# CPJKU/beat_this

Hardware: AMD Instinct MI355X
Metric: audio-seconds processed/sec (higher is better)
Workload: dtype f32 activations, f16x3 products (3 x f16 MFMA on hi+lo operand halves, f32 accumulate); main-layer attention P.V: 2 x, probabilities as fp16 hi parts

## Files before the change

### beat_this_amd/csrc/gemm3.hip

```cpp

#include "common.h"
#include "kernels.h"

struct G3CfgS { static constexpr int BM = 128, BN = 128, BK = 32, WGM = 2, WGN = 2, NST = 3, OCC = 3; };
struct G3CfgB { static constexpr int BM = 256, BN = 256, BK = 64, WGM = 2, WGN = 4, NST = 2, OCC = 1; };
struct G3CfgT { static constexpr int BM = 192, BN = 256, BK = 64, WGM = 2, WGN = 4, NST = 2, OCC = 1; };
struct G3CfgSX { static constexpr int BM = 128, BN = 128, BK = 64, WGM = 2, WGN = 2, NST = 2, OCC = 2; };
struct G3CfgBX { static constexpr int BM = 256, BN = 256, BK = 64, WGM = 2, WGN = 4, NST = 2, OCC = 1; };
struct G3CfgTX { static constexpr int BM = 192, BN = 256, BK = 64, WGM = 2, WGN = 4, NST = 2, OCC = 1; };
struct G3CfgMX { static constexpr int BM = 256, BN = 128, BK = 32, WGM = 2, WGN = 2, NST = 3, OCC = 2; };
struct G3CfgHX { static constexpr int BM = 64, BN = 128, BK = 64, WGM = 2, WGN = 2, NST = 3, OCC = 2; };

#ifndef X3_NSPLIT
#define X3_NSPLIT 2
#endif

namespace {

typedef G3CfgS CfgS;
typedef G3CfgB CfgB;

constexpr unsigned OOB = 0x80000000u;

#ifndef BT_NT_STORE
#define BT_NT_STORE 1
#endif
#if BT_NT_STORE
#define ST_STREAM(ptr, val) __builtin_nontemporal_store((val), (ptr))
#else
#define ST_STREAM(ptr, val) (*(ptr) = (val))
#endif

typedef __amdgpu_buffer_rsrc_t rsrc_t;
typedef __attribute__((address_space(3))) void* lptr_t;
typedef __attribute__((ext_vector_type(4))) unsigned int u32x4;
typedef __attribute__((ext_vector_type(2))) unsigned int u32x2;

DEVI unsigned pk2(float a, float b) {
  const hfx2 t = {(hf)a, (hf)b};
  return __builtin_bit_cast(unsigned, t);
}

DEVI void pack_row_hf(const float (&v)[16], u32x4 (&piece)[2]) {
#pragma unroll
  for (int k = 0; k < 2; ++k) {
    unsigned x0 = pk2(v[8 * k], v[8 * k + 1]), x1 = pk2(v[8 * k + 2], v[8 * k + 3]);
    unsigned y0 = pk2(v[8 * k + 4], v[8 * k + 5]), y1 = pk2(v[8 * k + 6], v[8 * k + 7]);
    auto r0 = __builtin_amdgcn_permlane32_swap(x0, y0, false, false);
    auto r1 = __builtin_amdgcn_permlane32_swap(x1, y1, false, false);
    piece[k] = u32x4{r0[0], r1[0], r0[1], r1[1]};
  }
}

DEVI void split2(float a, float b, unsigned& whi, unsigned& wlo, float& amax) {
  split_hl(a, b, whi, wlo);
  amax = fmaxf(amax, fmaxf(fabsf(a), fabsf(b)));
}
DEVI void pack_row_hl(const float (&v)[16], u32x4 (&hi)[2], u32x4 (&lo)[2], float& amax) {
#pragma unroll
  for (int k = 0; k < 2; ++k) {
    unsigned xh[2], xl[2], yh[2], yl[2];
    split2(v[8 * k], v[8 * k + 1], xh[0], xl[0], amax);
    split2(v[8 * k + 2], v[8 * k + 3], xh[1], xl[1], amax);
    split2(v[8 * k + 4], v[8 * k + 5], yh[0], yl[0], amax);
    split2(v[8 * k + 6], v[8 * k + 7], yh[1], yl[1], amax);
    auto h0 = __builtin_amdgcn_permlane32_swap(xh[0], yh[0], false, false);
    auto h1 = __builtin_amdgcn_permlane32_swap(xh[1], yh[1], false, false);
    auto l0 = __builtin_amdgcn_permlane32_swap(xl[0], yl[0], false, false);
    auto l1 = __builtin_amdgcn_permlane32_swap(xl[1], yl[1], false, false);
    hi[k] = u32x4{h0[0], h1[0], h0[1], h1[1]};
    lo[k] = u32x4{l0[0], l1[0], l0[1], l1[1]};
  }
}
DEVI void pack_row_f8(const float (&v)[16], u32x4 (&hi)[2], u32x2 (&h8)[2], u32x2 (&l8)[2], float& amax) {
#pragma unroll
  for (int k = 0; k < 2; ++k) {
    unsigned xh[2], xl[2], yh[2], yl[2];
    split2(v[8 * k], v[8 * k + 1], xh[0], xl[0], amax);
    split2(v[8 * k + 2], v[8 * k + 3], xh[1], xl[1], amax);
    split2(v[8 * k + 4], v[8 * k + 5], yh[0], yl[0], amax);
    split2(v[8 * k + 6], v[8 * k + 7], yh[1], yl[1], amax);
    const unsigned x8 = pk4_f8(v[8 * k], v[8 * k + 1], v[8 * k + 2], v[8 * k + 3]);
    const unsigned y8 = pk4_f8(v[8 * k + 4], v[8 * k + 5], v[8 * k + 6], v[8 * k + 7]);
    const unsigned xl8 = lo4_f8(v[8 * k], v[8 * k + 1], v[8 * k + 2], v[8 * k + 3], xh[0], xh[1]);
    const unsigned yl8 = lo4_f8(v[8 * k + 4], v[8 * k + 5], v[8 * k + 6], v[8 * k + 7], yh[0], yh[1]);
    auto h0 = __builtin_amdgcn_permlane32_swap(xh[0], yh[0], false, false);
    auto h1 = __builtin_amdgcn_permlane32_swap(xh[1], yh[1], false, false);
    auto b8 = __builtin_amdgcn_permlane32_swap(x8, y8, false, false);
    auto c8 = __builtin_amdgcn_permlane32_swap(xl8, yl8, false, false);
    hi[k] = u32x4{h0[0], h1[0], h0[1], h1[1]};
    h8[k] = u32x2{b8[0], b8[1]};
    l8[k] = u32x2{c8[0], c8[1]};
  }
}
DEVI void flag_range(int* status, float amax, float limit = 65504.f) {
  if (status && __any(!(amax <= limit)) && (threadIdx.x & 63) == 0) atomicOr(status, 1);
}

#ifndef BT_QKV_GATE_TILE
#define BT_QKV_GATE_TILE 1
#endif
template <typename CFG>
DEVI void qkv_gate_tile_x3(const Gemm3P& p, char* smem, int m0, int n0, int n_tiles, int lane, int wave) {
  constexpr int BM = CFG::BM, BN = CFG::BN, ROWB = CFG::BK * 2, NST = CFG::NST, KR = CFG::BK / 2, EB = 4;
  constexpr int NW = CFG::WGM * CFG::WGN, NT = 64 * NW;
  constexpr int CPR = ROWB / 16, RPI = 64 / CPR;
  constexpr int A_BYTES = BM * ROWB, ST_BYTES = A_BYTES + BN * ROWB;
  constexpr int APC = A_BYTES / (NT * 16), LPS = APC + 1;
  static_assert(ROWB == 128 && NW * 32 == BM && 32 * ROWB == NT * 16 && APC <= 4, "one 32-token block per wave, one W piece per thread");
  const int g = lane >> 5, lr = lane & 31;
  const int nk = p.K / KR;
  const int Lv = p.nblk * 32;
  auto swz = [](int r) { return (r >> 1) & 7; };
  const unsigned a_bytes = (unsigned)((long)p.M * p.lda * EB), w_bytes = (unsigned)((long)n_tiles * BN * p.K * EB);
  unsigned voffA[4];
#pragma unroll
  for (int i = 0; i < APC; ++i) {
    const int r = (i * NW + wave) * RPI + lane / CPR;
    const int c = (lane % CPR) ^ swz(r);
    const long row = (long)m0 + r;
    const int seq = (int)(row / Lv), t = (int)(row - (long)seq * Lv);
    voffA[i] = (seq < p.n_seq && t < p.L) ? (unsigned)(((long)seq * p.L + t) * p.lda * EB + c * 16) : OOB;
  }
  unsigned voffW;
  {
    const int r = wave * RPI + lane / CPR;
    voffW = (unsigned)((long)(n0 + r) * p.K * EB + ((lane % CPR) ^ swz(r)) * 16);
  }
  const rsrc_t rA = __builtin_amdgcn_make_buffer_rsrc(const_cast<char*>(reinterpret_cast<const char*>(p.A)), 0, a_bytes, 0x00020000);
  const rsrc_t rW = __builtin_amdgcn_make_buffer_rsrc(const_cast<void*>(p.W), 0, w_bytes, 0x00020000);
  auto issue = [&](int kt, int stage) {
    char* st_ = smem + stage * ST_BYTES + wave * 1024;
    const int so_ = kt * ROWB;
#pragma unroll
    for (int i_ = 0; i_ < APC; ++i_)
      __builtin_amdgcn_raw_ptr_buffer_load_lds(rA, (lptr_t)(st_ + i_ * NW * 1024), 16, voffA[i_], so_, 0, 0);
    __builtin_amdgcn_raw_ptr_buffer_load_lds(rW, (lptr_t)(st_ + A_BYTES), 16, voffW, so_, 0, 0);
  };
  const int pofs = A_BYTES + lr * ROWB;
  const int qofs = (wave * 32 + lr) * ROWB;
  const int sw = swz(lr);
  int kc[4];
#pragma unroll
  for (int m = 0; m < 4; ++m) kc[m] = ((2 * m + g) ^ sw) * 16;
  f32x16 acc;
#pragma unroll
  for (int r = 0; r < 16; ++r) acc[r] = 0.f;
  const int vb = m0 + wave * 32;
  const int tseq = vb / Lv, tblk = (vb - tseq * Lv) >> 5;
  const int t = tblk * 32 + lr;
  const long trow = (tseq < p.n_seq && t < p.L) ? (long)tseq * p.L + t : -1;
  float part[8];
#pragma unroll
  for (int q = 0; q < 8; ++q) part[q] = (p.ssq_in && trow >= 0 && q < p.ssq_parts) ? p.ssq_in[(long)q * p.M + trow] : 0.f;
#pragma unroll
  for (int s0 = 0; s0 < NST - 1; ++s0)
    if (s0 < nk) issue(s0, s0);
  asm volatile("s_waitcnt vmcnt(0)" ::: "memory");
  __builtin_amdgcn_sched_barrier(0);
  float rs = 1.f;
  if (p.ssq_in) {
    float sum = 0.f;
#pragma unroll
    for (int q = 0; q < 8; ++q) sum += part[q];
    for (int q = 8; q < p.ssq_parts; ++q) sum += trow >= 0 ? p.ssq_in[(long)q * p.M + trow] : 0.f;
    rs = trow >= 0 ? sqrtf((float)p.K) / fmaxf(sqrtf(sum), 1e-12f) : 0.f;
  }
  int stage = 0, stage2 = NST - 1;
  for (int kt = 0; kt < nk; ++kt) {
    if (NST > 2 && kt + 1 < nk) asm volatile("s_waitcnt vmcnt(%0) lgkmcnt(0)" ::"n"((NST - 2) * LPS) : "memory");
    else asm volatile("s_waitcnt vmcnt(0) lgkmcnt(0)" ::: "memory");
    __builtin_amdgcn_s_barrier();
    if (kt + NST - 1 < nk) issue(kt + NST - 1, stage2);
    const char* st = smem + stage * ST_BYTES;
#pragma unroll
    for (int m = 0; m < 2; ++m) {
      const hfx8 ph = *reinterpret_cast<const hfx8*>(st + pofs + kc[m]);
      const hfx8 pl = *reinterpret_cast<const hfx8*>(st + pofs + kc[m + 2]);
      const hfx8 qh = *reinterpret_cast<const hfx8*>(st + qofs + kc[m]);
      const hfx8 ql = *reinterpret_cast<const hfx8*>(st + qofs + kc[m + 2]);
      acc = MFMA32_H(pl, qh, acc);
      acc = MFMA32_H(ph, ql, acc);
      acc = MFMA32_H(ph, qh, acc);
    }
    stage = stage == NST - 1 ? 0 : stage + 1;
    stage2 = stage2 == NST - 1 ? 0 : stage2 + 1;
  }
  if (tseq >= p.n_seq) return;
#pragma unroll
  for (int r = 0; r < 16; ++r) {
    const int h = n0 - 3 * p.inner + crow(r, g);
    if (h < p.heads) p.gates[((long)tseq * p.heads + h) * p.nbp * 32 + t] = sigmoidf(fmaf(acc[r], rs, p.b_gates[h]));
  }
}

template <int EPI, typename CFG, int X3 = 0>
__global__ __launch_bounds__(64 * CFG::WGM * CFG::WGN, (CFG::OCC * CFG::WGM * CFG::WGN + 3) / 4)
void gemm3_kernel(const Gemm3P p, int n_tiles, int total_tiles, int per_xcd, int nsplit) {
  constexpr int BM = CFG::BM, BN = CFG::BN, BK = CFG::BK, NST = CFG::NST;
  constexpr int NW = CFG::WGM * CFG::WGN, NT = 64 * NW;
  constexpr int TB = BM / CFG::WGM / 32;
  constexpr int FB = BN / CFG::WGN / 32;
  constexpr int ROWB = BK * 2;
  constexpr int KR = X3 ? BK / 2 : BK;
  constexpr bool HL16 = X3 && BK == 32;
  constexpr int EB = X3 ? 4 : 2;
  constexpr int CPR = ROWB / 16;
  constexpr int RPI = 64 / CPR;
  constexpr int A_BYTES = BM * ROWB, W_BYTES = BN * ROWB, ST_BYTES = A_BYTES + W_BYTES;
  constexpr int APC = A_BYTES / (NT * 16), WPC = W_BYTES / (NT * 16);
  static_assert(EPI != G3_QKV || TB == FB, "the V columns swap the operand roles: square wave tile needed");
  static_assert(BN / CFG::WGN == 64, "ssq partials are per 64 columns = one wave");
  static_assert(!X3 || ROWB == 128 || ROWB == 64, "hl32: a k-step is a whole group (128 B per row) or half of one (64 B)");
  static_assert(X3 != 2 || ROWB == 128, "hl8: a k-step is a whole 32-column group");
  static_assert(NST * ST_BYTES >= NW * 8192, "the epilogues stage 8 KB per wave in the ring's LDS");
  __shared__ __attribute__((aligned(16))) char smem[NST * ST_BYTES];
  const int bid = blockIdx.x;
  int m_tile, n_tile;
  if (nsplit <= 1) {
    const int tile = (bid & 7) * per_xcd + (bid >> 3);
    if (tile >= total_tiles) return;
    m_tile = tile / n_tiles;
    n_tile = tile - m_tile * n_tiles;
  } else {
    const int xcd = bid & 7, slot = bid >> 3;
    const int g = xcd % nsplit, j = xcd / nsplit, per_m = 8 / nsplit, nt = n_tiles / nsplit;
    const int m_local = slot / nt;
    m_tile = m_local * per_m + j;
    n_tile = g * nt + (slot - m_local * nt);
    if ((long)m_tile * n_tiles >= total_tiles) return;
  }
  const int m0 = m_tile * BM, n0 = n_tile * BN;
  const int tid = threadIdx.x, lane = tid & 63, wave = __builtin_amdgcn_readfirstlane(tid >> 6);
  const int g = lane >> 5, lr = lane & 31;
  const int wm = wave / CFG::WGN, wn = wave % CFG::WGN;
  const int nk = p.K / KR;
  auto swz = [](int r) { return ROWB == 64 ? (r >> 2) & 3 : (r >> 1) & 7; };
  const int Lv = p.nblk * 32;

  int kind = 0;
  if constexpr (EPI == G3_QKV) kind = n0 < 3 * p.inner ? n0 / p.inner : 3;
  const bool normal = EPI == G3_QKV && kind == 2;
  if constexpr (BT_QKV_GATE_TILE && EPI == G3_QKV && X3 == 1 && BM == 128 && BN == 128 && ROWB == 128 && NW == 4) {
    if (kind == 3 && p.heads <= 32 && (p.x3 & 15) != 3) {
      qkv_gate_tile_x3<CFG>(p, smem, m0, n0, n_tiles, lane, wave);
      return;
    }
  }

  const unsigned a_bytes = (unsigned)((long)p.M * p.lda * EB), w_bytes = (unsigned)((long)n_tiles * BN * p.K * EB);
  static_assert(APC >= 1 && WPC >= 1, "tile too small for the workgroup");
  static_assert(APC <= 4 && WPC <= 4, "voffA / voffW hold at most 4 pieces");
  unsigned voffA[4], voffW[4];
  int tapmask[4] = {0, 0, 0, 0};
#pragma unroll
  for (int i = 0; i < APC; ++i) {
    const int r = (i * NW + wave) * RPI + lane / CPR;
    const int c = (lane % CPR) ^ swz(r);
    long row = (long)m0 + r;
    bool ok = row < p.M;
    if constexpr (EPI == G3_QKV) {
      const int seq = (int)(row / Lv), t = (int)(row - (long)seq * Lv);
      ok = seq < p.n_seq && t < p.L;
      row = (long)seq * p.L + t;
    }
    voffA[i] = ok ? (unsigned)(row * p.lda * EB + (HL16 ? (c >> 1) * 64 + (c & 1) * 16 : c * 16)) : OOB;
    if constexpr (EPI == G3_RESID) {
      const int t = p.conv_C2 > 0 ? (int)((row / p.conv_F) % p.conv_T) : 1;
      tapmask[i] = ok ? ((t >= 1 ? 1 : 0) | 2 | (t + 1 < p.conv_T ? 4 : 0)) : 0;
    }
  }
#pragma unroll
  for (int i = 0; i < WPC; ++i) {
    const int r = (i * NW + wave) * RPI + lane / CPR;
    const int c = (lane % CPR) ^ swz(r);
    voffW[i] = (unsigned)((long)(n0 + r) * p.K * EB + (HL16 ? (c >> 1) * 64 + (c & 1) * 16 : c * 16));
  }
  const bool conv = EPI == G3_RESID && p.conv_C2 > 0;
  const unsigned tap_bytes = conv ? (unsigned)(p.conv_F * p.conv_C2 * EB) : 0u;
  const int c2_shift = conv ? __builtin_ctz((unsigned)p.conv_C2) : 0;
  const rsrc_t rA = __builtin_amdgcn_make_buffer_rsrc(const_cast<char*>(reinterpret_cast<const char*>(p.A)) - tap_bytes, 0,
                                                      a_bytes + 2 * tap_bytes, 0x00020000);
  const rsrc_t rW = __builtin_amdgcn_make_buffer_rsrc(const_cast<void*>(p.W), 0, w_bytes, 0x00020000);
#define G3_ISSUE(kt, stage)                                                                                          \
  do {                                                                                                                \
    char* st_ = smem + (stage) * ST_BYTES + wave * 1024;                                                              \
    const int so_ = HL16 ? ((kt) >> 1) * 128 + ((kt) & 1) * 32 : (kt) * ROWB;                                         \
    if (conv) {                                                                                                       \
      const int tap_ = ((kt) * KR) >> c2_shift;                                                                       \
      const int kin_ = ((kt) * KR) & (p.conv_C2 - 1);                                                                 \
      const int soa_ = tap_ * (int)tap_bytes + (HL16 ? (kin_ >> 5) * 128 + ((kin_ >> 4) & 1) * 32 : kin_ * EB);      \
      _Pragma("unroll") for (int i_ = 0; i_ < APC; ++i_)                                                              \
          __builtin_amdgcn_raw_ptr_buffer_load_lds(rA, (lptr_t)(st_ + i_ * NW * 1024), 16,                            \
                                                   ((tapmask[i_] >> tap_) & 1) ? voffA[i_] : OOB, soa_, 0, 0);        \
    } else {                                                                                                          \
      _Pragma("unroll") for (int i_ = 0; i_ < APC; ++i_)                                                              \
          __builtin_amdgcn_raw_ptr_buffer_load_lds(rA, (lptr_t)(st_ + i_ * NW * 1024), 16, voffA[i_], so_, 0, 0);     \
    }                                                                                                                 \
    _Pragma("unroll") for (int i_ = 0; i_ < WPC; ++i_)                                                                \
        __builtin_amdgcn_raw_ptr_buffer_load_lds(rW, (lptr_t)(st_ + A_BYTES + i_ * NW * 1024), 16, voffW[i_], so_, 0, 0); \
  } while (0)

  constexpr int NP = FB, NQ = TB;
  const int pofs = (normal ? wm * (TB * 32) * ROWB : A_BYTES + wn * (FB * 32) * ROWB) + lr * ROWB;
  const int qofs = (normal ? A_BYTES + wn * (FB * 32) * ROWB : wm * (TB * 32) * ROWB) + lr * ROWB;
  const int sw = swz(lr);
  constexpr int MS = ROWB / 32;
  int kc[MS];
#pragma unroll
  for (int m = 0; m < MS; ++m) kc[m] = ((2 * m + g) ^ sw) * 16;

  f32x16 acc[NP][NQ];
#pragma unroll
  for (int a = 0; a < NP; ++a)
#pragma unroll
    for (int b = 0; b < NQ; ++b)
#pragma unroll
      for (int r = 0; r < 16; ++r) acc[a][b][r] = 0.f;

  const int row0 = m0 + wm * (TB * 32);
  long trow[TB];
  int tseq[TB], tblk[TB];
#pragma unroll
  for (int j = 0; j < TB; ++j) {
    const long v = (long)row0 + 32 * j + lr;
    if constexpr (EPI == G3_QKV) {
      const int vb = row0 + 32 * j;
      tseq[j] = vb / Lv;
      tblk[j] = (vb - tseq[j] * Lv) >> 5;
      const int t = tblk[j] * 32 + lr;
      trow[j] = (tseq[j] < p.n_seq && t < p.L) ? (long)tseq[j] * p.L + t : -1;
    } else {
      tseq[j] = tblk[j] = 0;
      trow[j] = v < p.M ? v : -1;
    }
  }
  float rs[TB], part[TB][8];
#pragma unroll
  for (int j = 0; j < TB; ++j) {
    rs[j] = 1.f;
#pragma unroll
    for (int q = 0; q < 8; ++q)
      part[j][q] = (EPI != G3_RESID && p.ssq_in && trow[j] >= 0 && q < p.ssq_parts) ? p.ssq_in[(long)q * p.M + trow[j]] : 0.f;
  }
  f32x4 bqv[EPI == G3_FF1 ? FB : 1][4];
  if constexpr (EPI == G3_FF1) {
#pragma unroll
    for (int a = 0; a < FB; ++a)
#pragma unroll
      for (int q = 0; q < 4; ++q) bqv[a][q] = *reinterpret_cast<const f32x4*>(p.bias + n0 + wn * 64 + a * 32 + 8 * q + 4 * g);
  }
  f32x4 csv[EPI == G3_QKV ? TB : 1][4];
  if constexpr (EPI == G3_QKV) {
    if (kind < 2) {
#pragma unroll
      for (int b = 0; b < TB; ++b)
#pragma unroll
        for (int q = 0; q < 4; ++q)
          csv[b][q] = tseq[b] < p.n_seq ? *reinterpret_cast<const f32x4*>(p.rope + ((long)(tblk[b] * 32 + lr) * 16 + 4 * q + 2 * g) * 2)
                                        : f32x4{0.f, 0.f, 0.f, 0.f};
    }
  }
  constexpr int LPS = APC + WPC;
#pragma unroll
  for (int s0 = 0; s0 < NST - 1; ++s0)
    if (s0 < nk) G3_ISSUE(s0, s0);
  if (EPI == G3_FF1 || EPI == G3_QKV || (EPI != G3_RESID && p.ssq_in)) {
    asm volatile("s_waitcnt vmcnt(0)" ::: "memory");
    __builtin_amdgcn_sched_barrier(0);
  }
  if (EPI != G3_RESID && p.ssq_in) {
#pragma unroll
    for (int j = 0; j < TB; ++j) {
      float sum = 0.f;
#pragma unroll
      for (int q = 0; q < 8; ++q) sum += part[j][q];
      for (int q = 8; q < p.ssq_parts; ++q) sum += trow[j] >= 0 ? p.ssq_in[(long)q * p.M + trow[j]] : 0.f;
      rs[j] = trow[j] >= 0 ? sqrtf((float)p.K) / fmaxf(sqrtf(sum), 1e-12f) : 0.f;
    }
  }
  int stage = 0, stage2 = NST - 1;
  for (int kt = 0; kt < nk; ++kt) {
    long long tq0 = 0, tq1 = 0;
    if (NST > 2 && kt + 1 < nk) asm volatile("s_waitcnt vmcnt(%0) lgkmcnt(0)" ::"n"((NST - 2) * LPS) : "memory");
    else asm volatile("s_waitcnt vmcnt(0) lgkmcnt(0)" ::: "memory");
    __builtin_amdgcn_s_barrier();
    if (kt + NST - 1 < nk) G3_ISSUE(kt + NST - 1, stage2);
    const char* st = smem + stage * ST_BYTES;
    if constexpr (X3 == 2) {
      typedef __attribute__((ext_vector_type(8))) int i32x8;
      const int cP = 4 + 2 * g, cQ = 6 - 2 * g;
      const int kP0 = (cP ^ sw) * 16, kP1 = ((cP + 1) ^ sw) * 16, kQ0 = (cQ ^ sw) * 16, kQ1 = ((cQ + 1) ^ sw) * 16;
      {
        i32x8 p8[NP], q8[NQ];
#pragma unroll
        for (int a = 0; a < NP; ++a) {
          const u32x4 lo = *reinterpret_cast<const u32x4*>(st + pofs + a * 32 * ROWB + kP0);
          const u32x4 hi = *reinterpret_cast<const u32x4*>(st + pofs + a * 32 * ROWB + kP1);
          p8[a] = i32x8{(int)lo[0], (int)lo[1], (int)lo[2], (int)lo[3], (int)hi[0], (int)hi[1], (int)hi[2], (int)hi[3]};
        }
#pragma unroll
        for (int b = 0; b < NQ; ++b) {
          const u32x4 lo = *reinterpret_cast<const u32x4*>(st + qofs + b * 32 * ROWB + kQ0);
          const u32x4 hi = *reinterpret_cast<const u32x4*>(st + qofs + b * 32 * ROWB + kQ1);
          q8[b] = i32x8{(int)lo[0], (int)lo[1], (int)lo[2], (int)lo[3], (int)hi[0], (int)hi[1], (int)hi[2], (int)hi[3]};
        }
#pragma unroll
        for (int a = 0; a < NP; ++a)
#pragma unroll
          for (int b = 0; b < NQ; ++b)
            acc[a][b] = __builtin_amdgcn_mfma_scale_f32_32x32x64_f8f6f4(p8[a], q8[b], acc[a][b], 0, 0, 0, HL8_SCALE_WORD, 0, 0x7f7f7f7f);
      }
#pragma unroll
      for (int m = 0; m < 2; ++m) {
        hfx8 ph[NP], qh[NQ];
#pragma unroll
        for (int a = 0; a < NP; ++a) ph[a] = *reinterpret_cast<const hfx8*>(st + pofs + a * 32 * ROWB + kc[m]);
#pragma unroll
        for (int b = 0; b < NQ; ++b) qh[b] = *reinterpret_cast<const hfx8*>(st + qofs + b * 32 * ROWB + kc[m]);
#pragma unroll
        for (int a = 0; a < NP; ++a)
#pragma unroll
          for (int b = 0; b < NQ; ++b) acc[a][b] = MFMA32_H(ph[a], qh[b], acc[a][b]);
      }
    } else if constexpr (!X3) {
#pragma unroll
      for (int m = 0; m < MS; ++m) {
        hfx8 fp[NP], fq[NQ];
#pragma unroll
        for (int a = 0; a < NP; ++a) fp[a] = *reinterpret_cast<const hfx8*>(st + pofs + a * 32 * ROWB + kc[m]);
#pragma unroll
        for (int b = 0; b < NQ; ++b) fq[b] = *reinterpret_cast<const hfx8*>(st + qofs + b * 32 * ROWB + kc[m]);
#pragma unroll
        for (int a = 0; a < NP; ++a)
#pragma unroll
          for (int b = 0; b < NQ; ++b) acc[a][b] = MFMA32_H(fp[a], fq[b], acc[a][b]);
      }
    } else {
#pragma unroll
      for (int m = 0; m < MS / 2; ++m) {
        hfx8 ph[NP], pl[NP], qh[NQ], ql[NQ];
#pragma unroll
        for (int a = 0; a < NP; ++a) {
          ph[a] = *reinterpret_cast<const hfx8*>(st + pofs + a * 32 * ROWB + kc[m]);
          pl[a] = *reinterpret_cast<const hfx8*>(st + pofs + a * 32 * ROWB + kc[m + MS / 2]);
        }
#pragma unroll
        for (int b = 0; b < NQ; ++b) {
          qh[b] = *reinterpret_cast<const hfx8*>(st + qofs + b * 32 * ROWB + kc[m]);
          ql[b] = *reinterpret_cast<const hfx8*>(st + qofs + b * 32 * ROWB + kc[m + MS / 2]);
        }
#pragma unroll
        for (int a = 0; a < NP; ++a)
#pragma unroll
          for (int b = 0; b < NQ; ++b) acc[a][b] = MFMA32_H(pl[a], qh[b], acc[a][b]);
#pragma unroll
        for (int a = 0; a < NP; ++a)
#pragma unroll
          for (int b = 0; b < NQ; ++b) acc[a][b] = MFMA32_H(ph[a], ql[b], acc[a][b]);
#pragma unroll
        for (int a = 0; a < NP; ++a)
#pragma unroll
          for (int b = 0; b < NQ; ++b) acc[a][b] = MFMA32_H(ph[a], qh[b], acc[a][b]);
      }
    }
    stage = stage == NST - 1 ? 0 : stage + 1;
    stage2 = stage2 == NST - 1 ? 0 : stage2 + 1;
  }

#undef G3_ISSUE
  __syncthreads();
  char* wst = smem + wave * 8192;
  float amax = 0.f;
  if constexpr (EPI == G3_FF1 && X3) {
    char* out8 = reinterpret_cast<char*>(p.out);
    const int nb0 = n0 + wn * 64;
    const int r4 = lane >> 4, cp = lane & 15;
#pragma unroll
    for (int b = 0; b < TB; ++b) {
#pragma unroll
      for (int a = 0; a < FB; ++a) {
        float v[16];
#pragma unroll
        for (int r = 0; r < 16; ++r) v[r] = gelu_erf(fmaf(acc[a][b][r], rs[b], bqv[a][r >> 2][r & 3]));
        if (p.x3 & G3_X3_OUT_F8) {
          u32x4 hi[2];
          u32x2 h8[2], l8[2];
          pack_row_f8(v, hi, h8, l8, amax);
#pragma unroll
          for (int k = 0; k < 2; ++k) {
            *reinterpret_cast<u32x4*>(wst + lr * 256 + (((8 * a + 2 * k + g) ^ (lr & 15)) << 4)) = hi[k];
            *reinterpret_cast<u32x2*>(wst + lr * 256 + (((8 * a + 4 + k) ^ (lr & 15)) << 4) + 8 * g) = h8[k];
            *reinterpret_cast<u32x2*>(wst + lr * 256 + (((8 * a + 6 + k) ^ (lr & 15)) << 4) + 8 * g) = l8[k];
          }
        } else {
        u32x4 hi[2], lo[2];
        pack_row_hl(v, hi, lo, amax);
#pragma unroll
        for (int k = 0; k < 2; ++k) {
          *reinterpret_cast<u32x4*>(wst + lr * 256 + (((8 * a + 2 * k + g) ^ (lr & 15)) << 4)) = hi[k];
          *reinterpret_cast<u32x4*>(wst + lr * 256 + (((8 * a + 4 + 2 * k + g) ^ (lr & 15)) << 4)) = lo[k];
        }
        }
      }
      static_assert(FB == 2, "row = 64 features = 256 B of hl32");
#pragma unroll
      for (int ps = 0; ps < 8; ++ps) {
        const int r = ps * 4 + r4;
        const u32x4 w = *reinterpret_cast<const u32x4*>(wst + r * 256 + (cp << 4));
        const long row = (long)row0 + 32 * b + r;
        if (row < p.M) ST_STREAM(reinterpret_cast<u32x4*>(out8 + (row * p.ldo + nb0) * 4 + ((cp ^ (r & 15)) << 4)), w);
      }
    }
  } else if constexpr (EPI == G3_FF1) {
    hf* out = reinterpret_cast<hf*>(p.out);
    const int nb0 = n0 + wn * 64;
#pragma unroll
    for (int b = 0; b < TB; ++b) {
#pragma unroll
      for (int a = 0; a < FB; ++a) {
        float v[16];
#pragma unroll
        for (int r = 0; r < 16; ++r) v[r] = gelu_tanh(fmaf(acc[a][b][r], rs[b], bqv[a][r >> 2][r & 3]));
        u32x4 piece[2];
        pack_row_hf(v, piece);
#pragma unroll
        for (int k = 0; k < 2; ++k)
          *reinterpret_cast<u32x4*>(wst + lr * 128 + (((4 * a + 2 * k + g) ^ (lr & 7)) << 4)) = piece[k];
      }
      static_assert(FB == 2, "row = 64 features = 128 B");
#pragma unroll
      for (int ps = 0; ps < 4; ++ps) {
        const int r = ps * 8 + (lane >> 3), cp = lane & 7;
        const u32x4 w = *reinterpret_cast<const u32x4*>(wst + r * 128 + (cp << 4));
        const long row = (long)row0 + 32 * b + r;
        if (row < p.M) *reinterpret_cast<u32x4*>(out + row * p.ldo + nb0 + ((cp ^ (r & 7)) << 3)) = w;
      }
    }
  } else if constexpr (EPI == G3_RESID) {
    hf* xb = reinterpret_cast<hf*>(p.xb);
    const int nb0 = n0 + wn * 64;
    if (nb0 < p.N) {
    if (p.bias) {
#pragma unroll
      for (int a = 0; a < FB; ++a)
#pragma unroll
        for (int q = 0; q < 4; ++q) {
          const f32x4 bb = *reinterpret_cast<const f32x4*>(p.bias + nb0 + a * 32 + 8 * q + 4 * g);
#pragma unroll
          for (int b = 0; b < TB; ++b)
#pragma unroll
            for (int i = 0; i < 4; ++i) acc[a][b][4 * q + i] += bb[i];
        }
    }
    const int r4 = lane >> 4, cp = lane & 15;
    const unsigned ldx = (unsigned)p.ldx;
    const unsigned off_lane = (unsigned)(row0 + r4) * ldx + (unsigned)nb0;
    unsigned colq[4];
#pragma unroll
    for (int q = 0; q < 4; ++q) colq[q] = (unsigned)((cp ^ (4 * q + r4)) << 2);
    const int rows_left = p.M - row0 - r4;
    if (p.gelu) {
#pragma unroll
      for (int a = 0; a < FB; ++a)
#pragma unroll
        for (int b = 0; b < TB; ++b)
#pragma unroll
          for (int r = 0; r < 16; ++r) acc[a][b][r] = X3 ? gelu_erf(acc[a][b][r]) : gelu_tanh(acc[a][b][r]);
    }
#pragma unroll
    for (int b = 0; b < TB; ++b) {
      f32x4 xv[8];
#pragma unroll
      for (int ps = 0; ps < 8; ++ps) {
        const unsigned off = off_lane + (unsigned)(32 * b + 4 * ps) * ldx + colq[ps & 3];
        xv[ps] = (32 * b + 4 * ps < rows_left && !p.no_resid && p.x) ? *reinterpret_cast<const f32x4*>(p.x + off)
                                                               : f32x4{0.f, 0.f, 0.f, 0.f};
      }
#pragma unroll
      for (int a = 0; a < FB; ++a)
#pragma unroll
        for (int q = 0; q < 4; ++q)
          *reinterpret_cast<f32x4*>(wst + lr * 256 + (((8 * a + 2 * q + g) ^ (lr & 15)) << 4)) =
              f32x4{acc[a][b][4 * q], acc[a][b][4 * q + 1], acc[a][b][4 * q + 2], acc[a][b][4 * q + 3]};
#pragma unroll
      for (int ps = 0; ps < 8; ++ps) {
        const int r = ps * 4 + r4;
        const unsigned off = off_lane + (unsigned)(32 * b + 4 * ps) * ldx + colq[ps & 3];
        const bool ok = 32 * b + 4 * ps < rows_left;
        f32x4 v = *reinterpret_cast<const f32x4*>(wst + r * 256 + (cp << 4));
#pragma unroll
        for (int i = 0; i < 4; ++i) v[i] += xv[ps][i];
        if (ok) {
          if (p.x) *reinterpret_cast<f32x4*>(p.x + off) = v;
          if constexpr (X3) {
            if (xb) {
              const unsigned f = (unsigned)nb0 + colq[ps & 3];
              unsigned wh[2], wl[2];
              split2(v[0], v[1], wh[0], wl[0], amax);
              split2(v[2], v[3], wh[1], wl[1], amax);
              hf* d = xb + (2u * off - (f & 31u));
              *reinterpret_cast<u32x2*>(d) = u32x2{wh[0], wh[1]};
              if (p.x3 & G3_X3_OUT_F8) {
                char* gb = reinterpret_cast<char*>(d) - (f & 31u);
                *reinterpret_cast<unsigned*>(gb + 64) = pk4_f8(v[0], v[1], v[2], v[3]);
                *reinterpret_cast<unsigned*>(gb + 96) = lo4_f8(v[0], v[1], v[2], v[3], wh[0], wh[1]);
              } else {
                *reinterpret_cast<u32x2*>(d + 32) = u32x2{wl[0], wl[1]};
              }
            }
          } else {
            if (xb) *reinterpret_cast<u32x2*>(xb + off) = u32x2{pk2(v[0], v[1]), pk2(v[2], v[3])};
          }
        }
        if (p.ssq_out) {
          float ssq = ok ? fmaf(v[0], v[0], fmaf(v[1], v[1], fmaf(v[2], v[2], v[3] * v[3]))) : 0.f;
#pragma unroll
          for (int o = 8; o > 0; o >>= 1) ssq += __shfl_xor(ssq, o);
          if (ok && cp == 0) p.ssq_out[(unsigned)(n0 / 64 + wn) * (unsigned)p.M + (unsigned)(row0 + 32 * b + r)] = ssq;
        }
      }
    }
    }
  } else {
    constexpr int BLK_E = X3 ? 2048 : 1024;
    if (kind < 2) {
      hf* dst = reinterpret_cast<hf*>(kind == 0 ? p.qf : p.kf);
#pragma unroll
      for (int b = 0; b < TB; ++b) {
        if (tseq[b] >= p.n_seq) continue;
        const f32x4 (&cs)[4] = csv[b];
#pragma unroll
        for (int a = 0; a < FB; ++a) {
          const int head = (n0 - kind * p.inner + wn * 64 + a * 32) >> 5;
          hf* blk = dst + (((long)tseq[b] * p.heads + head) * p.nbp + tblk[b]) * BLK_E;
#pragma unroll
          for (int q = 0; q < 4; ++q) {
            const float e0 = acc[a][b][4 * q] * rs[b], o0 = acc[a][b][4 * q + 1] * rs[b];
            const float e1 = acc[a][b][4 * q + 2] * rs[b], o1 = acc[a][b][4 * q + 3] * rs[b];
            const float r0 = e0 * cs[q][0] - o0 * cs[q][1], r1 = o0 * cs[q][0] + e0 * cs[q][1];
            const float r2 = e1 * cs[q][2] - o1 * cs[q][3], r3 = o1 * cs[q][2] + e1 * cs[q][3];
            if constexpr (X3) {
              unsigned wh[2], wl[2];
              split2(r0, r1, wh[0], wl[0], amax);
              split2(r2, r3, wh[1], wl[1], amax);
              ST_STREAM(reinterpret_cast<u32x2*>(blk + (q * 32 + lr) * 8 + 4 * g), (u32x2{wh[0], wh[1]}));
              ST_STREAM(reinterpret_cast<u32x2*>(blk + 1024 + (q * 32 + lr) * 8 + 4 * g), (u32x2{wl[0], wl[1]}));
            } else {
              *reinterpret_cast<u32x2*>(blk + (q * 32 + lr) * 8 + 4 * g) = u32x2{pk2(r0, r1), pk2(r2, r3)};
            }
          }
        }
      }
    } else if (kind == 2) {
      hf* dst = reinterpret_cast<hf*>(p.vf);
#pragma unroll
      for (int a = 0; a < TB; ++a) {
        if (tseq[a] >= p.n_seq) continue;
        float sk[16];
#pragma unroll
        for (int r = 0; r < 16; ++r) sk[r] = __shfl(rs[a], crow(r, g));
#pragma unroll
        for (int b = 0; b < FB; ++b) {
          const int head = (n0 - 2 * p.inner + wn * 64 + b * 32) >> 5;
          hf* blk = dst + (((long)tseq[a] * p.heads + head) * p.nbp + tblk[a]) * BLK_E;
#pragma unroll
          for (int s = 0; s < 2; ++s) {
            unsigned w[4], wl[4] = {0, 0, 0, 0};
#pragma unroll
            for (int i = 0; i < 4; ++i) {
              const float v0 = acc[a][b][8 * s + 2 * i] * sk[8 * s + 2 * i], v1 = acc[a][b][8 * s + 2 * i + 1] * sk[8 * s + 2 * i + 1];
              if constexpr (X3) split2(v0, v1, w[i], wl[i], amax);
              else w[i] = pk2(v0, v1);
            }
            ST_STREAM(reinterpret_cast<u32x4*>(blk + (s * 64 + lane) * 8), (u32x4{w[0], w[1], w[2], w[3]}));
            if constexpr (X3) ST_STREAM(reinterpret_cast<u32x4*>(blk + 1024 + (s * 64 + lane) * 8), (u32x4{wl[0], wl[1], wl[2], wl[3]}));
          }
        }
      }
    } else {
#pragma unroll
      for (int b = 0; b < TB; ++b) {
        if (tseq[b] >= p.n_seq) continue;
        const int t = tblk[b] * 32 + lr;
#pragma unroll
        for (int a = 0; a < FB; ++a)
#pragma unroll
          for (int r = 0; r < 16; ++r) {
            const int h = n0 - 3 * p.inner + wn * 64 + a * 32 + crow(r, g);
            if (h < p.heads)
              p.gates[((long)tseq[b] * p.heads + h) * p.nbp * 32 + t] = sigmoidf(fmaf(acc[a][b][r], rs[b], p.b_gates[h]));
          }
      }
    }
  }
  if constexpr (X3) flag_range(p.status, amax, (p.x3 & G3_X3_OUT_F8) ? HL8_ACT_MAX : 65504.f);
}

template <int EPI, typename CFG, int X3 = 0>
void launch_cfg(const Gemm3P& p, hipStream_t s) {
  const int n_tiles = (p.N + CFG::BN - 1) / CFG::BN;
  const long rows = p.epi == G3_QKV ? (long)p.n_seq * p.nblk * 32 : (long)p.M;
  const long m_tiles = (rows + CFG::BM - 1) / CFG::BM;
  const long total = m_tiles * n_tiles;
  int nsplit = (p.x3 >> 4) & 15;
  if (nsplit == 0) nsplit = (X3 && X3_NSPLIT > 1 && (long)n_tiles * CFG::BN * p.K * 4 > (5L << 19) && n_tiles % X3_NSPLIT == 0) ? X3_NSPLIT : 1;
  if (nsplit != 2 && nsplit != 4 && nsplit != 8) nsplit = 1;
  if (n_tiles % nsplit) nsplit = 1;
  long per;
  if (nsplit == 1) {
    per = (total + 7) / 8;
    per = (per + n_tiles - 1) / n_tiles * n_tiles;
  } else {
    const long per_m = 8 / nsplit;
    per = (m_tiles + per_m - 1) / per_m * (n_tiles / nsplit);
  }
  dim3 grid((unsigned)(per * 8)), block(64 * CFG::WGM * CFG::WGN);
  hipLaunchKernelGGL((gemm3_kernel<EPI, CFG, X3>), grid, block, 0, s, p, n_tiles, (int)total, (int)per, nsplit);
}

}

bool gemm3_supported(const Gemm3P& p) {
  const int eb = p.x3 ? 4 : 2;
  if (p.M <= 0 || p.K % 64 != 0 || p.K < 128 || p.lda % 8 != 0) return false;
  if ((long)p.M * p.lda * eb >= 0x7fffffffL || (long)(p.N + 255) / 256 * 256 * p.K * eb >= 0x7fffffffL) return false;
  if (p.x3 && BT_HALF_IS_BF16) return false;
  if (p.conv_C2 > 0 && (p.epi != G3_RESID || (p.conv_C2 & (p.conv_C2 - 1)) || p.conv_C2 % 32 != 0 || p.lda != p.conv_C2 ||
                        p.K != 3 * p.conv_C2 || p.conv_F <= 0 || p.conv_T <= 0 || p.M % (p.conv_T * p.conv_F) != 0 || !p.no_resid))
    return false;
  if (p.epi == G3_RESID && !p.x && !p.xb) return false;
  if (p.epi == G3_QKV) return p.inner % 128 == 0 && p.inner == p.heads * 32 && p.L > 0 && (long)p.n_seq * ((p.L + 31) / 32 * 32) < 0x7fffffffL;
  if (p.epi == G3_FF1) return p.N % 128 == 0 && p.ldo % 8 == 0;
  if (p.epi == G3_RESID) return p.N % 64 == 0 && p.ldx % 8 == 0 && (long)(p.M + 256) * p.ldx * (p.x3 ? 2 : 1) < 0x7fffffffL &&
                                (long)(p.N / 64) * p.M < 0x7fffffffL;
  return false;
}

#ifndef X3_BIG_FF1
#define X3_BIG_FF1 0
#endif
#ifndef X3_MX
#define X3_MX 1
#endif

int launch_gemm3(const Gemm3P& p, hipStream_t s) {
  if (!gemm3_supported(p)) return -2;
  const bool big_ok = p.epi != G3_QKV && p.N % 256 == 0;
  const int force = (p.x3 & 15) == 2 ? 1 : (p.x3 & 15) == 3 ? 0 : -1;
  const bool forced_small = (p.x3 & 15) == 4 || (p.x3 & 15) == 5;
  const long tiles192 = ((long)p.M + 191) / 192 * (p.N / 256);
  const bool fills = !p.x3 || tiles192 >= 160;
  const bool big = big_ok && !forced_small && (force == 1 || (force != 0 && p.epi == G3_RESID && p.K >= 1024 && p.M >= 4096 && fills) ||
                              (force != 0 && p.x3 && X3_BIG_FF1 && p.epi == G3_FF1 && p.M >= 4096));
  auto cost = [&](int bm) { const long t = ((long)p.M + bm - 1) / bm * (p.N / 256); return (t + 255) / 256 * bm; };
  const bool rows192 = big && p.epi == G3_RESID && force != 1 && cost(192) < cost(256);
  const long mx_tiles = ((long)p.M + 255) / 256 * ((p.N + 127) / 128);
  const bool f8 = (p.x3 & G3_X3_F8) != 0;
  const bool mx = p.x3 && !f8 && p.epi != G3_QKV && !big && !rows192 && force != 0 &&
                  ((p.x3 & 15) == 4 || (X3_MX && mx_tiles >= 512 && p.M >= 20000));
  const long sx_tiles = ((long)p.M + 127) / 128 * ((p.N + 127) / 128);
  const bool hx = p.x3 && p.epi == G3_RESID && !big && !rows192 && !mx &&
                  ((p.x3 & 15) == 5 || ((p.x3 & 15) <= 1 && (sx_tiles < 256 || (p.K < 1024 && p.M < 20000))));
  if (p.x3) {
    if (f8) {
      if (p.epi == G3_QKV) launch_cfg<G3_QKV, G3CfgSX, 2>(p, s);
      else if (p.epi == G3_FF1) { if (big) launch_cfg<G3_FF1, G3CfgBX, 2>(p, s); else launch_cfg<G3_FF1, G3CfgSX, 2>(p, s); }
      else if (hx) launch_cfg<G3_RESID, G3CfgHX, 2>(p, s);
      else if (rows192) launch_cfg<G3_RESID, G3CfgTX, 2>(p, s);
      else if (big) launch_cfg<G3_RESID, G3CfgBX, 2>(p, s);
      else launch_cfg<G3_RESID, G3CfgSX, 2>(p, s);
      return (int)hipGetLastError();
    }
    switch (p.epi) {
      case G3_FF1:
        if (mx) launch_cfg<G3_FF1, G3CfgMX, true>(p, s);
        else if (big) launch_cfg<G3_FF1, G3CfgBX, true>(p, s); else launch_cfg<G3_FF1, G3CfgSX, true>(p, s);
        break;
      case G3_RESID:
        if (mx) launch_cfg<G3_RESID, G3CfgMX, true>(p, s);
        else if (hx) launch_cfg<G3_RESID, G3CfgHX, true>(p, s);
        else if (rows192) launch_cfg<G3_RESID, G3CfgTX, true>(p, s);
        else if (big) launch_cfg<G3_RESID, G3CfgBX, true>(p, s);
        else launch_cfg<G3_RESID, G3CfgSX, true>(p, s);
        break;
      case G3_QKV: launch_cfg<G3_QKV, G3CfgSX, true>(p, s); break;
      default: return -1;
    }
    return (int)hipGetLastError();
  }
  switch (p.epi) {
    case G3_FF1:
      if (big) launch_cfg<G3_FF1, CfgB>(p, s);
      else launch_cfg<G3_FF1, CfgS>(p, s);
      break;
    case G3_RESID:
      if (rows192) launch_cfg<G3_RESID, G3CfgT>(p, s);
      else if (big) launch_cfg<G3_RESID, CfgB>(p, s);
      else launch_cfg<G3_RESID, CfgS>(p, s);
      break;
    case G3_QKV: launch_cfg<G3_QKV, CfgS>(p, s); break;
    default: return -1;
  }
  return (int)hipGetLastError();
}
```

Baseline: 63670.

## Add phased ping-pong main loop for big f16x3 GEMM tiles

Adds a phased main loop for the 256x256 and 192x256 hl32 GEMM configs. The two wave rows are offset by a barrier, and each k-step is split into four MFMA phases between barriers, with LDS reads and split global-to-LDS loads interleaved and MFMAs run at raised priority. Row blocks are interleaved across wave rows so each 64-row A piece is loaded per phase, and the epilogue row mapping changes to match. It also changes the dispatch heuristics: a new cost threshold for choosing 192-row tiles, FF1 can route to the phased configs, and the big-FF1 M threshold rises. This aims to overlap memory traffic and LDS reads with matrix math, at the cost of more barriers and tighter register and scheduling constraints.

Measured after the change: 64280 (median of 6 runs). About the same (+0.9%).

```diff
diff --git a/beat_this_amd/csrc/gemm3.hip b/beat_this_amd/csrc/gemm3.hip
--- a/beat_this_amd/csrc/gemm3.hip
+++ b/beat_this_amd/csrc/gemm3.hip
@@ -8,6 +8,11 @@
 struct G3CfgSX { static constexpr int BM = 128, BN = 128, BK = 64, WGM = 2, WGN = 2, NST = 2, OCC = 2; };
 struct G3CfgBX { static constexpr int BM = 256, BN = 256, BK = 64, WGM = 2, WGN = 4, NST = 2, OCC = 1; };
 struct G3CfgTX { static constexpr int BM = 192, BN = 256, BK = 64, WGM = 2, WGN = 4, NST = 2, OCC = 1; };
+struct G3CfgBP : G3CfgBX {};
+struct G3CfgTP : G3CfgTX {};
+template <typename CFG> struct G3Phased { static constexpr bool value = false; };
+template <> struct G3Phased<G3CfgBP> { static constexpr bool value = true; };
+template <> struct G3Phased<G3CfgTP> { static constexpr bool value = true; };
 struct G3CfgMX { static constexpr int BM = 256, BN = 128, BK = 32, WGM = 2, WGN = 2, NST = 3, OCC = 2; };
 struct G3CfgHX { static constexpr int BM = 64, BN = 128, BK = 64, WGM = 2, WGN = 2, NST = 3, OCC = 2; };
 
@@ -209,6 +214,10 @@
   constexpr int RPI = 64 / CPR;
   constexpr int A_BYTES = BM * ROWB, W_BYTES = BN * ROWB, ST_BYTES = A_BYTES + W_BYTES;
   constexpr int APC = A_BYTES / (NT * 16), WPC = W_BYTES / (NT * 16);
+  constexpr bool PH = G3Phased<CFG>::value;
+  static_assert(!PH || (X3 == 1 && ROWB == 128 && NST == 2 && CFG::WGM == 2 && CFG::WGN == 4 && FB == 2 && (TB == 3 || TB == 4) &&
+                        APC == TB && WPC == 4 && (EPI == G3_FF1 || EPI == G3_RESID)),
+                "phased loop: hl32 operands, 8 waves as 2 x 4, a 64-row A piece per token-block pair, FF1 / RESID");
   static_assert(EPI != G3_QKV || TB == FB, "the V columns swap the operand roles: square wave tile needed");
   static_assert(BN / CFG::WGN == 64, "ssq partials are per 64 columns = one wave");
   static_assert(!X3 || ROWB == 128 || ROWB == 64, "hl32: a k-step is a whole group (128 B per row) or half of one (64 B)");
@@ -318,12 +327,13 @@
 #pragma unroll
       for (int r = 0; r < 16; ++r) acc[a][b][r] = 0.f;
 
-  const int row0 = m0 + wm * (TB * 32);
+  const int row0 = PH ? m0 : m0 + wm * (TB * 32);
+  auto brow = [&](int b) { return PH ? 32 * (b < 2 ? 2 * wm + b : 4 + (TB - 2) * wm + (b - 2)) : 32 * b; };
   long trow[TB];
   int tseq[TB], tblk[TB];
 #pragma unroll
   for (int j = 0; j < TB; ++j) {
-    const long v = (long)row0 + 32 * j + lr;
+    const long v = (long)row0 + brow(j) + lr;
     if constexpr (EPI == G3_QKV) {
       const int vb = row0 + 32 * j;
       tseq[j] = vb / Lv;
@@ -362,10 +372,31 @@
     }
   }
   constexpr int LPS = APC + WPC;
+#define G3_ISSUE_A(kt, stage, i_)                                                                                     \
+  __builtin_amdgcn_raw_ptr_buffer_load_lds(rA, (lptr_t)(smem + (stage) * ST_BYTES + wave * 1024 + (i_) * NW * 1024), 16, voffA[i_], \
+                                           (kt) * ROWB, 0, 0)
+#define G3_ISSUE_W(kt, stage, i_)                                                                                     \
+  __builtin_amdgcn_raw_ptr_buffer_load_lds(rW, (lptr_t)(smem + (stage) * ST_BYTES + wave * 1024 + A_BYTES + (i_) * NW * 1024), 16, \
+                                           voffW[i_], (kt) * ROWB, 0, 0)
+  if constexpr (PH) {
+#pragma unroll
+    for (int i = 0; i < 2; ++i) G3_ISSUE_A(0, 0, i);
+#pragma unroll
+    for (int i = 0; i < 4; ++i) G3_ISSUE_W(0, 0, i);
+#pragma unroll
+    for (int i = 2; i < APC; ++i) G3_ISSUE_A(0, 0, i);
+    if (nk > 1) {
+#pragma unroll
+      for (int i = 0; i < 2; ++i) G3_ISSUE_A(1, 1, i);
+#pragma unroll
+      for (int i = 0; i < 4; ++i) G3_ISSUE_W(1, 1, i);
+    }
+  } else {
 #pragma unroll
   for (int s0 = 0; s0 < NST - 1; ++s0)
     if (s0 < nk) G3_ISSUE(s0, s0);
-  if (EPI == G3_FF1 || EPI == G3_QKV || (EPI != G3_RESID && p.ssq_in)) {
+  }
+  if (PH || EPI == G3_FF1 || EPI == G3_QKV || (EPI != G3_RESID && p.ssq_in)) {
     asm volatile("s_waitcnt vmcnt(0)" ::: "memory");
     __builtin_amdgcn_sched_barrier(0);
   }
@@ -379,6 +410,98 @@
       rs[j] = trow[j] >= 0 ? sqrtf((float)p.K) / fmaxf(sqrtf(sum), 1e-12f) : 0.f;
     }
   }
+  if constexpr (PH) {
+    constexpr int NL = APC - 2;
+    const int wofs = A_BYTES + (wn * 64 + lr) * ROWB;
+    int aofs[TB];
+#pragma unroll
+    for (int b = 0; b < TB; ++b) aofs[b] = (brow(b) + lr) * ROWB;
+    hfx8 wh[2][FB], wl[2][FB], qh[2][2], ql[2][2];
+    auto rd_w = [&](const char* st, int m) __attribute__((always_inline)) {
+#pragma unroll
+      for (int a = 0; a < FB; ++a) {
+        wh[m][a] = *reinterpret_cast<const hfx8*>(st + wofs + a * 32 * ROWB + kc[m]);
+        wl[m][a] = *reinterpret_cast<const hfx8*>(st + wofs + a * 32 * ROWB + kc[m + 2]);
+      }
+    };
+    auto rd_a = [&](const char* st, int h, int m) __attribute__((always_inline)) {
+#pragma unroll
+      for (int bb = 0; bb < 2; ++bb)
+        if (2 * h + bb < TB) {
+          qh[m][bb] = *reinterpret_cast<const hfx8*>(st + aofs[2 * h + bb] + kc[m]);
+          ql[m][bb] = *reinterpret_cast<const hfx8*>(st + aofs[2 * h + bb] + kc[m + 2]);
+        }
+    };
+    auto mm = [&](int h, int m) __attribute__((always_inline)) {
+      __builtin_amdgcn_sched_barrier(0);
+      asm volatile("s_waitcnt lgkmcnt(0)" ::: "memory");
+      __builtin_amdgcn_s_barrier();
+      __builtin_amdgcn_sched_barrier(0);
+      __builtin_amdgcn_s_setprio(1);
+#pragma unroll
+      for (int a = 0; a < FB; ++a)
+#pragma unroll
+        for (int bb = 0; bb < 2; ++bb)
+          if (2 * h + bb < TB) acc[a][2 * h + bb] = MFMA32_H(wl[m][a], qh[m][bb], acc[a][2 * h + bb]);
+#pragma unroll
+      for (int a = 0; a < FB; ++a)
+#pragma unroll
+        for (int bb = 0; bb < 2; ++bb)
+          if (2 * h + bb < TB) acc[a][2 * h + bb] = MFMA32_H(wh[m][a], ql[m][bb], acc[a][2 * h + bb]);
+#pragma unroll
+      for (int a = 0; a < FB; ++a)
+#pragma unroll
+        for (int bb = 0; bb < 2; ++bb)
+          if (2 * h + bb < TB) acc[a][2 * h + bb] = MFMA32_H(wh[m][a], qh[m][bb], acc[a][2 * h + bb]);
+      __builtin_amdgcn_s_setprio(0);
+      __builtin_amdgcn_sched_barrier(0);
+      __builtin_amdgcn_s_barrier();
+      __builtin_amdgcn_sched_barrier(0);
+    };
+    __builtin_amdgcn_s_barrier();
+    if (wm == 1) __builtin_amdgcn_s_barrier();
+    __builtin_amdgcn_sched_barrier(0);
+    rd_w(smem, 0);
+    rd_a(smem, 0, 0);
+    for (int kt = 0; kt < nk; ++kt) {
+      const int s = kt & 1;
+      const char* st = smem + s * ST_BYTES;
+      rd_w(st, 1);
+      rd_a(st, 0, 1);
+      if (kt + 1 < nk) {
+#pragma unroll
+        for (int i = 2; i < APC; ++i) G3_ISSUE_A(kt + 1, s ^ 1, i);
+        asm volatile("s_waitcnt vmcnt(%0)" ::"n"(APC + 4) : "memory");
+      } else {
+        asm volatile("s_waitcnt vmcnt(0)" ::: "memory");
+      }
+      mm(0, 0);
+      rd_a(st, 1, 0);
+      mm(0, 1);
+      rd_a(st, 1, 1);
+      if (kt + 2 < nk) {
+#pragma unroll
+        for (int i = 0; i < 2; ++i) G3_ISSUE_A(kt + 2, s, i);
+#pragma unroll
+        for (int i = 0; i < 2; ++i) G3_ISSUE_W(kt + 2, s, i);
+        asm volatile("s_waitcnt vmcnt(%0)" ::"n"(APC + 2) : "memory");
+      } else if (kt + 1 < nk) {
+        asm volatile("s_waitcnt vmcnt(%0)" ::"n"(NL) : "memory");
+      }
+      mm(1, 0);
+      if (kt + 1 < nk) {
+        rd_w(smem + (s ^ 1) * ST_BYTES, 0);
+        rd_a(smem + (s ^ 1) * ST_BYTES, 0, 0);
+      }
+      if (kt + 2 < nk) {
+#pragma unroll
+        for (int i = 2; i < 4; ++i) G3_ISSUE_W(kt + 2, s, i);
+      }
+      mm(1, 1);
+    }
+    asm volatile("s_waitcnt lgkmcnt(0)" ::: "memory");
+    if (wm == 0) __builtin_amdgcn_s_barrier();
+  } else {
   int stage = 0, stage2 = NST - 1;
   for (int kt = 0; kt < nk; ++kt) {
     long long tq0 = 0, tq1 = 0;
@@ -467,8 +590,11 @@
     stage = stage == NST - 1 ? 0 : stage + 1;
     stage2 = stage2 == NST - 1 ? 0 : stage2 + 1;
   }
+  }
 
 #undef G3_ISSUE
+#undef G3_ISSUE_A
+#undef G3_ISSUE_W
   __syncthreads();
   char* wst = smem + wave * 8192;
   float amax = 0.f;
@@ -508,7 +634,7 @@
       for (int ps = 0; ps < 8; ++ps) {
         const int r = ps * 4 + r4;
         const u32x4 w = *reinterpret_cast<const u32x4*>(wst + r * 256 + (cp << 4));
-        const long row = (long)row0 + 32 * b + r;
+        const long row = (long)row0 + brow(b) + r;
         if (row < p.M) ST_STREAM(reinterpret_cast<u32x4*>(out8 + (row * p.ldo + nb0) * 4 + ((cp ^ (r & 15)) << 4)), w);
       }
     }
@@ -573,8 +699,8 @@
       f32x4 xv[8];
 #pragma unroll
       for (int ps = 0; ps < 8; ++ps) {
-        const unsigned off = off_lane + (unsigned)(32 * b + 4 * ps) * ldx + colq[ps & 3];
-        xv[ps] = (32 * b + 4 * ps < rows_left && !p.no_resid && p.x) ? *reinterpret_cast<const f32x4*>(p.x + off)
+        const unsigned off = off_lane + (unsigned)(brow(b) + 4 * ps) * ldx + colq[ps & 3];
+        xv[ps] = (brow(b) + 4 * ps < rows_left && !p.no_resid && p.x) ? *reinterpret_cast<const f32x4*>(p.x + off)
                                                                : f32x4{0.f, 0.f, 0.f, 0.f};
       }
 #pragma unroll
@@ -586,8 +712,8 @@
 #pragma unroll
       for (int ps = 0; ps < 8; ++ps) {
         const int r = ps * 4 + r4;
-        const unsigned off = off_lane + (unsigned)(32 * b + 4 * ps) * ldx + colq[ps & 3];
-        const bool ok = 32 * b + 4 * ps < rows_left;
+        const unsigned off = off_lane + (unsigned)(brow(b) + 4 * ps) * ldx + colq[ps & 3];
+        const bool ok = brow(b) + 4 * ps < rows_left;
         f32x4 v = *reinterpret_cast<const f32x4*>(wst + r * 256 + (cp << 4));
 #pragma unroll
         for (int i = 0; i < 4; ++i) v[i] += xv[ps][i];
@@ -617,7 +743,7 @@
           float ssq = ok ? fmaf(v[0], v[0], fmaf(v[1], v[1], fmaf(v[2], v[2], v[3] * v[3]))) : 0.f;
 #pragma unroll
           for (int o = 8; o > 0; o >>= 1) ssq += __shfl_xor(ssq, o);
-          if (ok && cp == 0) p.ssq_out[(unsigned)(n0 / 64 + wn) * (unsigned)p.M + (unsigned)(row0 + 32 * b + r)] = ssq;
+          if (ok && cp == 0) p.ssq_out[(unsigned)(n0 / 64 + wn) * (unsigned)p.M + (unsigned)(row0 + brow(b) + r)] = ssq;
         }
       }
     }
@@ -743,18 +869,24 @@
 #ifndef X3_MX
 #define X3_MX 1
 #endif
+#ifndef X3_PHASED
+#define X3_PHASED 1
+#endif
 
 int launch_gemm3(const Gemm3P& p, hipStream_t s) {
   if (!gemm3_supported(p)) return -2;
   const bool big_ok = p.epi != G3_QKV && p.N % 256 == 0;
-  const int force = (p.x3 & 15) == 2 ? 1 : (p.x3 & 15) == 3 ? 0 : -1;
+  const int fc = p.x3 & 15;
+  const int force = (fc == 2 || fc == 6 || fc == 7) ? 1 : fc == 3 ? 0 : -1;
   const bool forced_small = (p.x3 & 15) == 4 || (p.x3 & 15) == 5;
   const long tiles192 = ((long)p.M + 191) / 192 * (p.N / 256);
   const bool fills = !p.x3 || tiles192 >= 160;
   const bool big = big_ok && !forced_small && (force == 1 || (force != 0 && p.epi == G3_RESID && p.K >= 1024 && p.M >= 4096 && fills) ||
-                              (force != 0 && p.x3 && X3_BIG_FF1 && p.epi == G3_FF1 && p.M >= 4096));
+                              (force != 0 && p.x3 && X3_BIG_FF1 && p.epi == G3_FF1 && p.M >= 20000));
   auto cost = [&](int bm) { const long t = ((long)p.M + bm - 1) / bm * (p.N / 256); return (t + 255) / 256 * bm; };
-  const bool rows192 = big && p.epi == G3_RESID && force != 1 && cost(192) < cost(256);
+  const bool phased = p.x3 && !(p.x3 & G3_X3_F8) && p.conv_C2 == 0 && (fc == 6 || fc == 7 || (fc != 2 && X3_PHASED));
+  const bool fewer192 = phased ? cost(192) * 8 < cost(256) * 7 : cost(192) < cost(256);
+  const bool rows192 = big && (fc == 7 || (p.epi == G3_RESID && force != 1 && fewer192));
   const long mx_tiles = ((long)p.M + 255) / 256 * ((p.N + 127) / 128);
   const bool f8 = (p.x3 & G3_X3_F8) != 0;
   const bool mx = p.x3 && !f8 && p.epi != G3_QKV && !big && !rows192 && force != 0 &&
@@ -775,12 +907,16 @@
     switch (p.epi) {
       case G3_FF1:
         if (mx) launch_cfg<G3_FF1, G3CfgMX, true>(p, s);
+        else if (rows192) launch_cfg<G3_FF1, G3CfgTP, true>(p, s);
+        else if (big && phased) launch_cfg<G3_FF1, G3CfgBP, true>(p, s);
         else if (big) launch_cfg<G3_FF1, G3CfgBX, true>(p, s); else launch_cfg<G3_FF1, G3CfgSX, true>(p, s);
         break;
       case G3_RESID:
         if (mx) launch_cfg<G3_RESID, G3CfgMX, true>(p, s);
         else if (hx) launch_cfg<G3_RESID, G3CfgHX, true>(p, s);
+        else if (rows192 && phased) launch_cfg<G3_RESID, G3CfgTP, true>(p, s);
         else if (rows192) launch_cfg<G3_RESID, G3CfgTX, true>(p, s);
+        else if (big && phased) launch_cfg<G3_RESID, G3CfgBP, true>(p, s);
         else if (big) launch_cfg<G3_RESID, G3CfgBX, true>(p, s);
         else launch_cfg<G3_RESID, G3CfgSX, true>(p, s);
         break;
```
